# BenLangmead/bowtie2

Hardware: NVIDIA H100
Metric: Mreads/s (higher is better)
Workload: dtype u64 popcount (FM rank) + s16x2 DPX (DP)

## Files before the change

### bowtie2_b200/csrc/fm_device.cuh

```cuda
#pragma once
#include "bt2g_internal.h"

#define BT2G_OFFMASK (~(uint64_t)0)

template <typename OFF> struct SideGeom;
template <> struct SideGeom<uint32_t> {
	static constexpr uint32_t SIDE_SZ = 64, BWT_SZ = 48, BWT_LEN = 192, WORDS = 6, VECS = 4;
};
template <> struct SideGeom<uint64_t> {
	static constexpr uint32_t SIDE_SZ = 128, BWT_SZ = 96, BWT_LEN = 384, WORDS = 12, VECS = 8;
};

template <typename OFF>
struct SideRegs {
	uint64_t w[SideGeom<OFF>::WORDS];
	uint64_t occ[4];
};

__device__ __forceinline__ void ldg_sector(const uint8_t *p, uint64_t &a, uint64_t &b, uint64_t &c, uint64_t &d) {
	asm volatile("ld.global.nc.L1::no_allocate.L2::64B.v2.u64 {%0,%1}, [%4];\n\t"
	             "ld.global.nc.L1::no_allocate.L2::64B.v2.u64 {%2,%3}, [%4+16];"
	             : "=l"(a), "=l"(b), "=l"(c), "=l"(d) : "l"(p));
}
__device__ __forceinline__ void ldg_sector128(const uint8_t *p, uint64_t &a, uint64_t &b, uint64_t &c, uint64_t &d) {
// ... 203 lines not shown
		if((uint64_t)refl >= start && (uint64_t)(refl + ncol) <= start + (uint64_t)ix.recLen[lo]) {
			fast = true;
			b0 = ix.recCumUnamb[lo] + ((uint64_t)refl - start);
		}
	}
	if(fast) {
		for(int k = lane; k < ncol; k += 32) {
			const uint64_t b = b0 + (uint64_t)k;
			out[k] = (uint8_t)((ix.refBuf[b >> 2] >> ((b & 3) << 1)) & 3);
		}
	} else {
		for(int k = lane; k < ncol; k += 32) out[k] = (uint8_t)ref_base<OFF>(ix, tidx, refl + k);
	}
}

__device__ __forceinline__ int read_char(const uint8_t *seq, int len, int strand, int pos) {
	if(strand == 0) return seq[pos];
	int c = seq[len - 1 - pos];
	return c > 3 ? 4 : 3 - c;
}

template <typename OFF>
__device__ __forceinline__ uint32_t extend_one(const DevEbwt<OFF> &e, uint64_t top, uint64_t bot, const uint8_t *s, int len,
                                               int strand, int i0, int step, int lim) {
	uint32_t n = 0;
	for(int ii = 0; ii < lim; ii++) {
		const int rdc = read_char(s, len, strand, i0 + ii * step);
		if(bot - top > 1) {
			uint64_t t[4], b[4];
			rank4<OFF>(e, top, t);
			rank4<OFF>(e, bot, b);
			const uint64_t orig = bot - top;
			int nonz = -1; bool abort = false;
#pragma unroll
			for(int j = 0; j < 4; j++) {
				if(!abort && b[j] > t[j]) {
					if(nonz >= 0) abort = true;
					else { nonz = j; top = t[j]; bot = b[j]; }
				}
			}
			if(abort || (nonz != rdc && rdc <= 3) || bot - top < orig) break;
		} else {
			int c = -1;
			if(top != e.zOff) top = lf_step<OFF>(e, top, c);
			if(c != rdc && rdc <= 3) break;
			bot = top + 1;
		}
		if(++n == 255) break;
	}
	return n;
}

template <typename OFF>
__device__ __forceinline__ uint32_t extend_one_text(const DevIndex<OFF> &ix, int64_t b, int tstep, const uint8_t *s, int len,
                                                    int strand, int i0, int step, int lim) {
	uint32_t n = 0;
	const int64_t tlen = (int64_t)ix.fw.len;
	for(int ii = 0; ii < lim; ii++) {
		const int rdc = read_char(s, len, strand, i0 + ii * step);
		int c = -1;
		if(b >= 0 && b < tlen) { c = (int)((__ldg(ix.refBuf + (b >> 2)) >> ((b & 3) << 1)) & 3); b += tstep; }
		if(c != rdc && rdc <= 3) break;
		if(++n == 255) break;
	}
	return n;
}
__device__ __forceinline__ uint64_t swap_rev_pairs(uint64_t x) {
	const uint64_t y = __brevll(x);
	return ((y & 0x5555555555555555ull) << 1) | ((y >> 1) & 0x5555555555555555ull);
}
__device__ __forceinline__ uint64_t spread_bits(uint32_t m) {
	uint64_t x = m;
	x = (x | (x << 16)) & 0x0000ffff0000ffffull;
	x = (x | (x << 8)) & 0x00ff00ff00ff00ffull;
	x = (x | (x << 4)) & 0x0f0f0f0f0f0f0f0full;
	x = (x | (x << 2)) & 0x3333333333333333ull;
	x = (x | (x << 1)) & 0x5555555555555555ull;
	return x;
}
template <typename F>
__device__ __forceinline__ uint64_t walk_window(F word, int64_t p, bool asc, int64_t n, uint32_t &ok) {
	int64_t q = asc ? p : p - 31;
	int lshift = 0;
	if(q < 0) { lshift = (int)(-q); q = 0; }
	uint64_t a = 0;
	if(lshift < 32 && q < n) {
		const int64_t w = q >> 5; const int sh = (int)(q & 31);
		a = word(w) >> (2 * sh);
		if(sh && ((w + 1) << 5) < n) a |= word(w + 1) << (64 - 2 * sh);
		if(lshift) a <<= 2 * lshift;
	}
	const int64_t q0 = asc ? p : p - 31;
	uint32_t v = 0xffffffffu;
	if(q0 < 0) v = q0 <= -32 ? 0u : (v << (int)(-q0));
	if(q0 + 32 > n) { const int64_t keep = n - q0; v = keep <= 0 ? 0u : (keep >= 32 ? v : (v & ((1u << (int)keep) - 1u))); }
	if(asc) { ok = v; return a; }
	ok = __brev(v);
	return swap_rev_pairs(a);
}
template <typename OFF>
__device__ __forceinline__ uint32_t extend_one_text_packed(const DevIndex<OFF> &ix, int64_t b, int tstep, const uint64_t *pk, const uint32_t *nm, int len,
                                                           int strand, int i0, int step, int lim) {
	const int64_t tlen = (int64_t)ix.fw.len;
	const uint64_t *tw = reinterpret_cast<const uint64_t *>(ix.refBuf);
	auto tword = [&](int64_t k) -> uint64_t { return __ldg(tw + k); };
	auto rword = [&](int64_t k) -> uint64_t { return pk[k]; };
	int64_t rp = strand == 0 ? i0 : len - 1 - i0;
	const bool rasc = strand == 0 ? step > 0 : step < 0;
	const uint64_t comp = strand == 0 ? 0ull : ~0ull;
	int n = 0;
	if(lim > 255) lim = 255;
	while(n < lim) {
		uint32_t okR, okT, okN;
		const uint64_t R = walk_window(rword, rp, rasc, (int64_t)len, okR) ^ comp;
		const uint64_t T = walk_window(tword, b, tstep > 0, tlen, okT);
		uint32_t nmk;
		{
			int64_t q = rasc ? rp : rp - 31; int lshift = 0;
			if(q < 0) { lshift = (int)(-q); q = 0; }
			uint32_t a = 0;
			if(lshift < 32 && q < len) {
				const int64_t w = q >> 5; const int sh = (int)(q & 31);
				a = nm[w] >> sh;
				if(sh && ((w + 1) << 5) < len) a |= nm[w + 1] << (32 - sh);
				if(lshift) a <<= lshift;
			}
			nmk = rasc ? a : __brev(a);
			okN = 0;
		}
		(void)okN;
		const uint64_t X = R ^ T;
		const uint64_t neq = (X | (X >> 1)) & 0x5555555555555555ull;
		const uint64_t stop = (neq | spread_bits(~okT)) & ~spread_bits(nmk);
		const int chunk = lim - n < 32 ? lim - n : 32;
		int first = stop ? (__ffsll((long long)stop) - 1) >> 1 : 32;
		if(first < chunk) { n += first; break; }
		n += chunk;
		rp += rasc ? 32 : -32;
		b += tstep > 0 ? 32 : -32;
		(void)okR;
	}
	return (uint32_t)n;
}

template <typename OFF>
__device__ __forceinline__ void extend_hit(const DevIndex<OFF> &ix, const uint64_t rng[4], const uint8_t *s, int len, bool fw, int off, int sl,
                                           bool left, bool right, uint32_t &nlex, uint32_t &nrex, const uint64_t *pk = nullptr, const uint32_t *nm = nullptr) {
	const int strand = fw ? 0 : 1;
	const int limL = fw ? off : len - sl - off, limR = fw ? len - sl - off : off;
	const int i0L = fw ? off - 1 : len - off - sl - 1, i0R = fw ? sl + off : len - off;
	nlex = nrex = 0;
	const bool unique = ix.extText && ix.refBuf != nullptr && rng[1] - rng[0] == 1;
	int64_t p = 0;
	if(unique && ((left && limL > 0) || (right && limR > 0))) { unsigned ns = 0; p = (int64_t)get_offset<OFF>(ix, rng[0], ns); }
	if(left && limL > 0)
		nlex = !unique ? extend_one<OFF>(ix.fw, rng[0], rng[1], s, len, strand, i0L, -1, limL)
		     : (pk ? extend_one_text_packed<OFF>(ix, p - 1, -1, pk, nm, len, strand, i0L, -1, limL) : extend_one_text<OFF>(ix, p - 1, -1, s, len, strand, i0L, -1, limL));
	if(right && limR > 0 && ix.bw.ebwt != nullptr)
		nrex = !unique ? extend_one<OFF>(ix.bw, rng[2], rng[3], s, len, strand, i0R, +1, limR)
		     : (pk ? extend_one_text_packed<OFF>(ix, p + sl, +1, pk, nm, len, strand, i0R, +1, limR) : extend_one_text<OFF>(ix, p + sl, +1, s, len, strand, i0R, +1, limR));
}
```

### bowtie2_b200/csrc/fm_seed2.cu

```cuda
#include "fm_device.cuh"
#include <cstdlib>

#define REFILL_MIN 8

__global__ void k_pack_reads(const uint8_t *seq, const uint64_t *roff, uint64_t nReads, int maxWords,
                             uint64_t *packed, uint32_t *nmask) {
	uint64_t t = blockIdx.x * (uint64_t)blockDim.x + threadIdx.x;
	if(t >= nReads * (uint64_t)maxWords) return;
	const uint64_t rd = t / maxWords;
	const int w = (int)(t - rd * maxWords);
	const int len = (int)(roff[rd + 1] - roff[rd]);
	if(w * 32 >= len) return;
	const uint8_t *s = seq + roff[rd] + (uint64_t)w * 32;
	const int n = len - w * 32 < 32 ? len - w * 32 : 32;
	uint64_t p = 0; uint32_t m = 0;
	for(int i = 0; i < n; i++) {
		const uint32_t c = s[i];
		if(c > 3) m |= 1u << i; else p |= (uint64_t)c << (2 * i);
	}
	const uint64_t wb = (roff[rd] >> 5) + rd + (uint64_t)w;
	packed[wb] = p; nmask[wb] = m;
}

__device__ __forceinline__ uint64_t rev_pairs(uint64_t x, int n) {
	uint64_t r = __brevll(x);
	r = ((r >> 1) & 0x5555555555555555ull) | ((r & 0x5555555555555555ull) << 1);
	return r >> (64 - 2 * n);
}

template <typename OFF>
__device__ __forceinline__ void rank4_loaded(const DevEbwt<OFF> &e, const SideRegs<OFF> &s, uint64_t sideNum, uint32_t charOff, uint64_t out[4]) {
	uint32_t nC, nG, nT;
	count_cgt<OFF>(s, charOff, nC, nG, nT);
	uint32_t nA = charOff - nC - nG - nT;
	if(sideNum == e.zSide && charOff > e.zChar) nA--;
	out[0] = nA + s.occ[0] + e.fchr[0];
	out[1] = nC + s.occ[1] + e.fchr[1];
	out[2] = nG + s.occ[2] + e.fchr[2];
	out[3] = nT + s.occ[3] + e.fchr[3];
}

template <typename OFF>
__global__ void __launch_bounds__(256) k_seed_search2(DevIndex<OFF> ix, const uint64_t *packed, const uint32_t *nmask,
                                                      const uint64_t *roff, uint64_t nReads, int seedLen, int maxSeeds,
                                                      int nofw, int norc, const int32_t *interval, const int32_t *offset,
                                                      uint64_t *out, int32_t *nseedsOut, unsigned long long *next,
                                                      unsigned long long *cnt) {
	constexpr uint32_t BL = SideGeom<OFF>::BWT_LEN;
	const unsigned FULL = 0xffffffffu;
	const int lane = threadIdx.x & 31;
	const uint64_t perRead = 2ull * maxSeeds, total = nReads * perRead;
	const DevEbwt<OFF> &fw = ix.fw;
	const DevEbwt<OFF> &bw = ix.bw;
	const int ftabLen = fw.ftabChars;
	bool active = false, exhausted = false;
	uint64_t topf = 0, botf = 0, topb = 0, botb = 0, bits = 0;
	uint64_t *o = nullptr;
	int sl = 0, step = 0;
	unsigned nside = 0;
	for(;;) {
		const unsigned need = __ballot_sync(FULL, !active && !exhausted);
		if(need && (__popc(need) >= REFILL_MIN || __ballot_sync(FULL, active) == 0)) {
			unsigned long long base = 0;
			const int leader = __ffs(need) - 1;
			if(lane == leader) base = atomicAdd(next, (unsigned long long)__popc(need));
			base = __shfl_sync(FULL, base, leader);
			if(!active && !exhausted) {
				const uint64_t t = base + (unsigned)__popc(need & ((1u << lane) - 1u));
				if(t >= total) {
					exhausted = true;
				} else {
					const uint64_t rd = t / perRead;
					const int rem = (int)(t - rd * perRead);
					const int strand = rem / maxSeeds, k = rem - strand * maxSeeds;
					o = out + t * 4;
					reinterpret_cast<uint4 *>(o)[0] = make_uint4(0, 0, 0, 0);
					reinterpret_cast<uint4 *>(o)[1] = make_uint4(0, 0, 0, 0);
					const uint64_t r0 = roff[rd];
					const int len = (int)(roff[rd + 1] - r0);
					const int per = interval[rd], off0 = offset[rd];
					int nseeds = 1;
					if(len - off0 > seedLen) nseeds += (len - off0 - seedLen) / per;
					if(rem == 0 && nseedsOut) nseedsOut[rd] = nseeds;
					sl = seedLen < len ? seedLen : len;
					const int depth = k * per + off0;
					bool ok = k < nseeds && !((strand == 0 && nofw) || (strand == 1 && norc)) && depth + sl <= len && sl >= 1;
					if(ok) {
						const uint64_t wb = (r0 >> 5) + rd;
						const int w = depth >> 5, sh = depth & 31;
						const bool two = sh + sl > 32;
						const uint64_t p0 = packed[wb + w], p1 = two ? packed[wb + w + 1] : 0;
						const uint64_t n0 = nmask[wb + w], n1 = two ? nmask[wb + w + 1] : 0;
						const uint64_t m2 = sl == 32 ? ~0ull : ((1ull << (2 * sl)) - 1);
						bits = (sh ? ((p0 >> (2 * sh)) | (p1 << (64 - 2 * sh))) : p0) & m2;
						const uint64_t nb = ((n0 | (n1 << 32)) >> sh) & (sl == 32 ? 0xffffffffull : ((1ull << sl) - 1));
						if(nb) ok = false;
						if(strand == 1) bits = rev_pairs(bits, sl) ^ m2;
					}
					if(ok) {
						if(ix.ktab != nullptr && ix.ktabChars <= sl) {
							const OFF *e3 = ix.ktab + 3ull * (bits >> (2 * (sl - ix.ktabChars)));
							topf = e3[0]; botf = e3[1]; topb = e3[2]; botb = topb + (botf - topf);
							if(botf <= topf) ok = false;
							step = ix.ktabChars;
						} else if(ftabLen > 1 && ftabLen <= sl) {
							const uint64_t top20 = bits >> (2 * (sl - ftabLen));
							const uint64_t fwi = rev_pairs(top20, ftabLen), bwi = top20;
							topf = ftab_hi<OFF>(fw, fwi); botf = ftab_lo<OFF>(fw, fwi + 1);
							if(botf <= topf) ok = false;
							else if(bw.ebwt != nullptr) { topb = ftab_hi<OFF>(bw, bwi); botb = topb + (botf - topf); }
							else { topb = botb = 0; }
							step = ftabLen;
						} else {
							const int c = (int)((bits >> (2 * (sl - 1))) & 3);
							topf = topb = fw.fchr[c]; botf = botb = fw.fchr[c + 1];
							if(botf <= topf) ok = false;
							step = 1;
						}
					}
					if(ok) {
						if(step >= sl) { o[0] = topf; o[1] = botf; o[2] = topb; o[3] = botb; }
						else active = true;
					}
				}
			}
		}
		if(__ballot_sync(FULL, active) == 0) {
			if(__all_sync(FULL, exhausted)) break;
			continue;
		}
		if(active) {
			const int c = (int)((bits >> (2 * (sl - step - 1))) & 3);
			const uint64_t sideT = topf / BL, sideB = botf / BL;
			const uint32_t offT = (uint32_t)(topf - sideT * BL), offB = (uint32_t)(botf - sideB * BL);
			nside += (botf - topf > 1) ? 2 : 1;
			uint64_t tt[4], bb[4];
			SideRegs<OFF> s;
			load_side<OFF>(fw.ebwt, sideT, s);
			rank4_loaded<OFF>(fw, s, sideT, offT, tt);
			if(sideB != sideT) load_side<OFF>(fw.ebwt, sideB, s);
			rank4_loaded<OFF>(fw, s, sideB, offB, bb);
			const uint64_t w0 = bb[0] - tt[0], w1 = bb[1] - tt[1], w2 = bb[2] - tt[2];
			const uint64_t tp = topb + (c > 0 ? w0 : 0) + (c > 1 ? w1 : 0) + (c > 2 ? w2 : 0);
			const uint64_t nt = c == 0 ? tt[0] : (c == 1 ? tt[1] : (c == 2 ? tt[2] : tt[3]));
			const uint64_t nb = c == 0 ? bb[0] : (c == 1 ? bb[1] : (c == 2 ? bb[2] : bb[3]));
			if(nb <= nt) {
				active = false;
			} else {
				topf = nt; botf = nb; topb = tp; botb = tp + (nb - nt);
				if(++step == sl) { o[0] = topf; o[1] = botf; o[2] = topb; o[3] = botb; active = false; }
			}
		}
	}
	if(cnt && nside) atomicAdd(cnt, (unsigned long long)nside);
}

template <typename OFF>
__global__ void __launch_bounds__(256) k_seed_search3(DevIndex<OFF> ix, const uint64_t *packed, const uint32_t *nmask,
                                                      const uint64_t *roff, uint64_t nReads, int seedLen, int maxSeeds,
                                                      int nofw, int norc, const int32_t *interval, const int32_t *offset,
                                                      uint64_t *out, int32_t *nseedsOut, unsigned long long *next,
                                                      unsigned long long *cnt, const uint8_t *actv) {
	constexpr uint32_t BL = SideGeom<OFF>::BWT_LEN;
	const unsigned FULL = 0xffffffffu;
	const int lane = threadIdx.x & 31;
	const uint64_t total = nReads * 2;
	const DevEbwt<OFF> &fw = ix.fw;
	const DevEbwt<OFF> &bw = ix.bw;
	const int ftabLen = fw.ftabChars;
	bool haveTask = false, exhausted = false, active = false, skip = false;
	uint64_t topf = 0, botf = 0, topb = 0, botb = 0, bits = 0, wb = 0;
	uint64_t *o = nullptr, *obase = nullptr;
	int sl = 0, step = 0, k = 0, nseeds = 0, per = 1, off0 = 0, len = 0, strand = 0;
	unsigned nside = 0;
	for(;;) {
		const unsigned need = __ballot_sync(FULL, !haveTask && !exhausted);
		if(need && (__popc(need) >= REFILL_MIN || __ballot_sync(FULL, haveTask) == 0)) {
			unsigned long long base = 0;
			const int leader = __ffs(need) - 1;
			if(lane == leader) base = atomicAdd(next, (unsigned long long)__popc(need));
			base = __shfl_sync(FULL, base, leader);
			if(!haveTask && !exhausted) {
				const uint64_t t = base + (unsigned)__popc(need & ((1u << lane) - 1u));
				if(t >= total) exhausted = true;
				else if(actv && !actv[t >> 1]) { }
				else {
					const uint64_t rd = t >> 1;
					strand = (int)(t & 1);
					skip = (strand == 0 ? nofw : norc) || (actv && ((actv[rd] >> (1 + strand)) & 1));
					const uint64_t r0 = roff[rd];
					len = (int)(roff[rd + 1] - r0);
					per = interval[rd]; off0 = offset[rd];
					nseeds = 1;
					if(len - off0 > seedLen) nseeds += (len - off0 - seedLen) / per;
					if(strand == 0 && nseedsOut) nseedsOut[rd] = nseeds;
					sl = seedLen < len ? seedLen : len;
					wb = (r0 >> 5) + rd;
					obase = out + (rd * 2ull + strand) * (uint64_t)maxSeeds * 4;
					k = 0; haveTask = true; active = false;
				}
			}
		}
		if(__ballot_sync(FULL, haveTask) == 0) {
			if(__all_sync(FULL, exhausted)) break;
			continue;
		}
		if(haveTask && !active) {
			if(k >= maxSeeds) haveTask = false;
			else {
				o = obase + (uint64_t)k * 4;
				reinterpret_cast<uint4 *>(o)[0] = make_uint4(0, 0, 0, 0);
				reinterpret_cast<uint4 *>(o)[1] = make_uint4(0, 0, 0, 0);
				const int depth = k * per + off0;
				bool ok = k < nseeds && !skip && depth + sl <= len && sl >= 1;
				if(ok) {
					const int w = depth >> 5, sh = depth & 31;
					const bool two = sh + sl > 32;
					const uint64_t p0 = packed[wb + w], p1 = two ? packed[wb + w + 1] : 0;
					const uint64_t n0 = nmask[wb + w], n1 = two ? nmask[wb + w + 1] : 0;
					const uint64_t m2 = sl == 32 ? ~0ull : ((1ull << (2 * sl)) - 1);
					bits = (sh ? ((p0 >> (2 * sh)) | (p1 << (64 - 2 * sh))) : p0) & m2;
					const uint64_t nb = ((n0 | (n1 << 32)) >> sh) & (sl == 32 ? 0xffffffffull : ((1ull << sl) - 1));
					if(nb) ok = false;
					if(strand == 1) bits = rev_pairs(bits, sl) ^ m2;
				}
				if(ok) {
					if(ix.ktab != nullptr && ix.ktabChars <= sl) {
						const OFF *e3 = ix.ktab + 3ull * (bits >> (2 * (sl - ix.ktabChars)));
						topf = e3[0]; botf = e3[1]; topb = e3[2]; botb = topb + (botf - topf);
						if(botf <= topf) ok = false;
						step = ix.ktabChars;
					} else if(ftabLen > 1 && ftabLen <= sl) {
						const uint64_t top20 = bits >> (2 * (sl - ftabLen));
						const uint64_t fwi = rev_pairs(top20, ftabLen), bwi = top20;
						topf = ftab_hi<OFF>(fw, fwi); botf = ftab_lo<OFF>(fw, fwi + 1);
						if(botf <= topf) ok = false;
						else if(bw.ebwt != nullptr) { topb = ftab_hi<OFF>(bw, bwi); botb = topb + (botf - topf); }
						else { topb = botb = 0; }
						step = ftabLen;
					} else {
						const int c = (int)((bits >> (2 * (sl - 1))) & 3);
						topf = topb = fw.fchr[c]; botf = botb = fw.fchr[c + 1];
						if(botf <= topf) ok = false;
						step = 1;
					}
				}
				if(ok) {
					if(step >= sl) { o[0] = topf; o[1] = botf; o[2] = topb; o[3] = botb; }
					else active = true;
				}
				k++;
				if(!active && k >= nseeds) {
					for(; k < maxSeeds; k++) {
						uint64_t *z = obase + (uint64_t)k * 4;
						reinterpret_cast<uint4 *>(z)[0] = make_uint4(0, 0, 0, 0);
						reinterpret_cast<uint4 *>(z)[1] = make_uint4(0, 0, 0, 0);
					}
					haveTask = false;
				}
			}
		}
		if(active) {
			const int c = (int)((bits >> (2 * (sl - step - 1))) & 3);
			const uint64_t sideT = topf / BL, sideB = botf / BL;
			const uint32_t offT = (uint32_t)(topf - sideT * BL), offB = (uint32_t)(botf - sideB * BL);
			nside += (botf - topf > 1) ? 2 : 1;
			uint64_t tt[4], bb[4];
			SideRegs<OFF> s;
			load_side<OFF>(fw.ebwt, sideT, s);
			rank4_loaded<OFF>(fw, s, sideT, offT, tt);
			if(sideB != sideT) load_side<OFF>(fw.ebwt, sideB, s);
			rank4_loaded<OFF>(fw, s, sideB, offB, bb);
			const uint64_t w0 = bb[0] - tt[0], w1 = bb[1] - tt[1], w2 = bb[2] - tt[2];
			const uint64_t tp = topb + (c > 0 ? w0 : 0) + (c > 1 ? w1 : 0) + (c > 2 ? w2 : 0);
			const uint64_t nt = c == 0 ? tt[0] : (c == 1 ? tt[1] : (c == 2 ? tt[2] : tt[3]));
			const uint64_t nb = c == 0 ? bb[0] : (c == 1 ? bb[1] : (c == 2 ? bb[2] : bb[3]));
			if(nb <= nt) {
				active = false;
			} else {
				topf = nt; botf = nb; topb = tp; botb = tp + (nb - nt);
				if(++step == sl) { o[0] = topf; o[1] = botf; o[2] = topb; o[3] = botb; active = false; }
			}
		}
	}
	if(cnt && nside) atomicAdd(cnt, (unsigned long long)nside);
}

template <typename OFF>
void launch_seed_search2(const DevIndex<OFF> &ix, const uint8_t *seq, const uint64_t *roff, uint64_t nReads, int maxLen,
                         int seedLen, int maxSeeds, int nofw, int norc, const int32_t *interval, const int32_t *offset,
                         uint64_t *out, int32_t *nseeds, uint64_t *packed, uint32_t *nmask, unsigned long long *next,
                         int numSMs, cudaStream_t st, unsigned long long *cnt) {
	if(nReads == 0) return;
	(void)seq; (void)maxLen;
	cudaMemsetAsync(next, 0, sizeof(unsigned long long), st);
	int perSM = 4;
	const char *v2 = getenv("BT2G_SEED_V2");
	if(v2 && v2[0] == '1') {
		cudaOccupancyMaxActiveBlocksPerMultiprocessor(&perSM, k_seed_search2<OFF>, 256, 0);
		if(perSM < 1) perSM = 1;
		k_seed_search2<OFF><<<(unsigned)(numSMs * perSM), 256, 0, st>>>(ix, packed, nmask, roff, nReads, seedLen, maxSeeds, nofw, norc,
		                                                              interval, offset, out, nseeds, next, cnt);
		return;
	}
	cudaOccupancyMaxActiveBlocksPerMultiprocessor(&perSM, k_seed_search3<OFF>, 256, 0);
	if(perSM < 1) perSM = 1;
	k_seed_search3<OFF><<<(unsigned)(numSMs * perSM), 256, 0, st>>>(ix, packed, nmask, roff, nReads, seedLen, maxSeeds, nofw, norc,
	                                                              interval, offset, out, nseeds, next, cnt, nullptr);
}
template <typename OFF>
void launch_seed_search_active(const DevIndex<OFF> &ix, const uint64_t *roff, uint64_t nReads, int seedLen, int maxSeeds,
                               const int32_t *interval, const int32_t *offset, const uint8_t *actv, uint64_t *out, int32_t *nseeds,
                               const uint64_t *packed, const uint32_t *nmask, unsigned long long *next, int numSMs, cudaStream_t st) {
	if(nReads == 0) return;
	cudaMemsetAsync(next, 0, sizeof(unsigned long long), st);
	int perSM = 4;
	cudaOccupancyMaxActiveBlocksPerMultiprocessor(&perSM, k_seed_search3<OFF>, 256, 0);
	if(perSM < 1) perSM = 1;
	uint64_t blocks = (uint64_t)numSMs * perSM, want = (nReads * 2 + 255) / 256;
	if(want < blocks) blocks = want ? want : 1;
	k_seed_search3<OFF><<<(unsigned)blocks, 256, 0, st>>>(ix, packed, nmask, roff, nReads, seedLen, maxSeeds, 0, 0, interval, offset, out, nseeds, next, nullptr, actv);
}
template void launch_seed_search_active<uint32_t>(const DevIndex<uint32_t> &, const uint64_t *, uint64_t, int, int, const int32_t *, const int32_t *, const uint8_t *, uint64_t *, int32_t *, const uint64_t *, const uint32_t *, unsigned long long *, int, cudaStream_t);
template void launch_seed_search_active<uint64_t>(const DevIndex<uint64_t> &, const uint64_t *, uint64_t, int, int, const int32_t *, const int32_t *, const uint8_t *, uint64_t *, int32_t *, const uint64_t *, const uint32_t *, unsigned long long *, int, cudaStream_t);
template void launch_seed_search2<uint32_t>(const DevIndex<uint32_t> &, const uint8_t *, const uint64_t *, uint64_t, int, int, int, int, int, const int32_t *, const int32_t *, uint64_t *, int32_t *, uint64_t *, uint32_t *, unsigned long long *, int, cudaStream_t, unsigned long long *);
template void launch_seed_search2<uint64_t>(const DevIndex<uint64_t> &, const uint8_t *, const uint64_t *, uint64_t, int, int, int, int, int, const int32_t *, const int32_t *, uint64_t *, int32_t *, uint64_t *, uint32_t *, unsigned long long *, int, cudaStream_t, unsigned long long *);

template <typename OFF>
__global__ void k_build_ktab(DevIndex<OFF> ix, int K, OFF *out) {
	constexpr uint32_t BL = SideGeom<OFF>::BWT_LEN;
	const uint64_t x = blockIdx.x * (uint64_t)blockDim.x + threadIdx.x;
	if(x >> (2 * K)) return;
	const DevEbwt<OFF> &fw = ix.fw;
	const DevEbwt<OFF> &bw = ix.bw;
	const int F = fw.ftabChars;
	OFF *o = out + 3ull * x;
	o[0] = 0; o[1] = 0; o[2] = 0;
	const uint64_t top20 = x >> (2 * (K - F));
	const uint64_t fwi = rev_pairs(top20, F), bwi = top20;
	uint64_t topf = ftab_hi<OFF>(fw, fwi), botf = ftab_lo<OFF>(fw, fwi + 1);
	if(botf <= topf) return;
	uint64_t topb = ftab_hi<OFF>(bw, bwi);
	for(int step = F; step < K; step++) {
		const int c = (int)((x >> (2 * (K - step - 1))) & 3);
		const uint64_t sideT = topf / BL, sideB = botf / BL;
		const uint32_t offT = (uint32_t)(topf - sideT * BL), offB = (uint32_t)(botf - sideB * BL);
		uint64_t tt[4], bb[4];
		SideRegs<OFF> s;
		load_side<OFF>(fw.ebwt, sideT, s);
		rank4_loaded<OFF>(fw, s, sideT, offT, tt);
		if(sideB != sideT) load_side<OFF>(fw.ebwt, sideB, s);
		rank4_loaded<OFF>(fw, s, sideB, offB, bb);
		const uint64_t w0 = bb[0] - tt[0], w1 = bb[1] - tt[1], w2 = bb[2] - tt[2];
		const uint64_t tp = topb + (c > 0 ? w0 : 0) + (c > 1 ? w1 : 0) + (c > 2 ? w2 : 0);
		const uint64_t nt = c == 0 ? tt[0] : (c == 1 ? tt[1] : (c == 2 ? tt[2] : tt[3]));
		const uint64_t nb = c == 0 ? bb[0] : (c == 1 ? bb[1] : (c == 2 ? bb[2] : bb[3]));
		if(nb <= nt) return;
		topf = nt; botf = nb; topb = tp;
	}
	o[0] = (OFF)topf; o[1] = (OFF)botf; o[2] = (OFF)topb;
}

template <typename OFF>
void launch_build_ktab(const DevIndex<OFF> &ix, int K, OFF *out, cudaStream_t st) {
	const uint64_t n = 1ull << (2 * K);
	k_build_ktab<OFF><<<(unsigned)((n + 255) / 256), 256, 0, st>>>(ix, K, out);
}
template void launch_build_ktab<uint32_t>(const DevIndex<uint32_t> &, int, uint32_t *, cudaStream_t);
template void launch_build_ktab<uint64_t>(const DevIndex<uint64_t> &, int, uint64_t *, cudaStream_t);

template <typename OFF>
__global__ void k_build_dense_sa(DevIndex<OFF> ix, int rate, uint64_t entries, OFF *out) {
	const uint64_t i = blockIdx.x * (uint64_t)blockDim.x + threadIdx.x;
	if(i >= entries) return;
	DevIndex<OFF> base = ix;
	base.saOffs = ix.offs; base.saRate = ix.offRate;
	unsigned nside = 0;
	const uint64_t row = i << rate;
	out[i] = row < ix.fw.len + 1 ? (OFF)get_offset<OFF>(base, row, nside) : (OFF)0;
}

template <typename OFF>
void launch_build_dense_sa(const DevIndex<OFF> &ix, int rate, OFF *out, cudaStream_t st) {
	const uint64_t entries = ((ix.fw.len + 1) + ((1ull << rate) - 1)) >> rate;
	if(entries == 0) return;
	k_build_dense_sa<OFF><<<(unsigned)((entries + 255) / 256), 256, 0, st>>>(ix, rate, entries, out);
}
template void launch_build_dense_sa<uint32_t>(const DevIndex<uint32_t> &, int, uint32_t *, cudaStream_t);
template void launch_build_dense_sa<uint64_t>(const DevIndex<uint64_t> &, int, uint64_t *, cudaStream_t);

__device__ __forceinline__ int packed_char(const uint64_t *pk, const uint32_t *nm, uint64_t wb, int pos) {
	const int w = pos >> 5, b = pos & 31;
	if((nm[wb + w] >> b) & 1u) return 4;
	return (int)((pk[wb + w] >> (2 * b)) & 3);
}

template <typename OFF>
__device__ __forceinline__ uint32_t count_one(const SideRegs<OFF> &s, uint32_t charOff, int c) {
	const uint64_t M = 0x5555555555555555ull, pat = (uint64_t)c * M;
	const uint32_t wi = charOff >> 5, rem = charOff & 31;
	uint32_t n = 0;
#pragma unroll
	for(uint32_t i = 0; i < SideGeom<OFF>::WORDS; i++) {
		const uint64_t mask = i < wi ? M : (i == wi ? ((1ull << (2 * rem)) - 1) & M : 0);
		const uint64_t z = ~(s.w[i] ^ pat);
		n += __popcll(z & (z >> 1) & mask);
	}
	return n;
}

template <typename OFF>
__device__ __forceinline__ uint64_t rank1_loaded(const DevEbwt<OFF> &e, const SideRegs<OFF> &s, uint64_t sideNum, uint32_t charOff, int c) {
	uint32_t n = count_one<OFF>(s, charOff, c);
	if(c == 0 && sideNum == e.zSide && charOff > e.zChar) n--;
	const uint64_t oc = c == 0 ? s.occ[0] : (c == 1 ? s.occ[1] : (c == 2 ? s.occ[2] : s.occ[3]));
	return n + oc + e.fchr[c];
}

template <typename OFF>
__global__ void __launch_bounds__(256) k_exact_sweep2(DevIndex<OFF> ix, const uint64_t *packed, const uint32_t *nmask,
                                                      const uint64_t *roff, uint64_t nReads, int nofw, int norc,
                                                      uint8_t *mine, uint64_t *ee, unsigned long long *next, unsigned long long *cnt,
                                                      int flags) {
	const int eeOnly = flags & 1;
	const bool text = (flags & 2) != 0 && ix.refBuf != nullptr;
	constexpr uint32_t BL = SideGeom<OFF>::BWT_LEN;
	const unsigned FULL = 0xffffffffu;
	const int lane = threadIdx.x & 31;
	const uint64_t total = nReads * 2;
	const DevEbwt<OFF> &e = ix.fw;
	const int ftabLen = e.ftabChars;
	const int mineMax = 2;
	bool active = false, exhausted = false, doInit = true;
	uint64_t top = 0, bot = 0, wb = 0, task = 0;
	int len = 0, dep = 0, nedit = 0, strand = 0;
	int cacheW = -1; uint64_t cacheP = 0; uint32_t cacheM = 0;
	unsigned nside = 0;
	for(;;) {
		const unsigned need = __ballot_sync(FULL, !active && !exhausted);
		if(need && (__popc(need) >= REFILL_MIN || __ballot_sync(FULL, active) == 0)) {
			unsigned long long base = 0;
			const int leader = __ffs(need) - 1;
			if(lane == leader) base = atomicAdd(next, (unsigned long long)__popc(need));
			base = __shfl_sync(FULL, base, leader);
			if(!active && !exhausted) {
				cacheW = -1;
				task = base + (unsigned)__popc(need & ((1u << lane) - 1u));
				if(task >= total) exhausted = true;
				else {
					const uint64_t rd = task >> 1;
					strand = (int)(task & 1);
					if((strand == 0 && nofw) || (strand == 1 && norc)) {
						mine[task] = 0; ee[rd * 4 + strand * 2] = 0; ee[rd * 4 + strand * 2 + 1] = 0;
					} else {
						const uint64_t r0 = roff[rd];
						len = (int)(roff[rd + 1] - r0);
						wb = (r0 >> 5) + rd;
						dep = 0; nedit = 0; doInit = true; top = bot = 0;
						active = true;
						if(len <= 0) { mine[task] = 0; ee[rd * 4 + strand * 2] = 0; ee[rd * 4 + strand * 2 + 1] = 0; active = false; }
					}
				}
			}
		}
		if(__ballot_sync(FULL, active) == 0) {
			if(__all_sync(FULL, exhausted)) break;
			continue;
		}
		if(active) {
			bool done = false;
			auto rawchr = [&](int pos) -> int {
				const int w = pos >> 5, b = pos & 31;
				if(w != cacheW) { cacheW = w; cacheP = packed[wb + w]; cacheM = nmask[wb + w]; }
				if((cacheM >> b) & 1u) return 4;
// ... 190 lines not shown
```

### bowtie2_b200/csrc/xengine.cuh

```cuda
#pragma once
#include <stdint.h>
#include "../../include/bt2g.h"
#include "mapq_device.cuh"
#include "pe_device.cuh"

#ifndef XE_HD
#define XE_HD __host__ __device__
#endif
#define XE_HH __host__ __device__

namespace xe {

#define XE_MIN_I64 (-9223372036854775807LL - 1)
#define XE_BIG ((int64_t)1 << 62)
enum { EXHAUSTED = 1, FULFILLED, PERFECT, SOFT_LIMIT, HARD_LIMIT };
enum { XR_DONE = 0, XR_ONE_MM = 1, XR_SEED = 2, XR_DP = 3, XR_DP_MATE = 4, XR_FALLBACK = 5 };

#define XE_MAX_LEN    512
#define XE_ARENA      12288
#define XE_SEEN_IV    224
#define XE_EXR        8
#define XE_MM1        24
#define XE_MAX_SEEDS  64
#define XE_SATS       (2 * XE_MAX_SEEDS)
// ... 402 lines not shown
	}
	const int64_t sc = x_aln(u, a)->score;
	if(sc > u.usBest) { u.usBest2 = u.usBest; u.usBest = sc; } else if(sc > u.usBest2) u.usBest2 = sc;
	return u.usDone != 0;
}

XE_HD inline int64_t x_tightened(const XUnit &u, int64_t bestPairScore) {
	int64_t ps = u.best2Pair + ((u.bestPair - u.best2Pair) * 3) / 4;
	if(ps < bestPairScore) ps++;
	return ps;
}

template <typename Svc>
struct XEngine {
	const XParams &P; XUnit &u; Svc &svc;
	XE_HD XEngine(const XParams &p, XUnit &unit, Svc &s) : P(p), u(unit), svc(s) {}

	XE_HD int64_t mapq(int64_t best, bool hasSec, int64_t sec, int64_t scMin, int64_t perfect) const {
		if(!P.mmode && !hasSec) return 255;
		return mapq_v2(best, hasSec, sec, scMin, perfect, !P.local);
	}

	XE_HD int64_t shSize(const XMate &c, bool fw, int i) const { const uint64_t *h = svc.seedRange(c.idx, fw ? 0 : 1, i); return h[1] > h[0] ? (int64_t)(h[1] - h[0]) : 0; }
	XE_HD void fillSeedHits(XMate &c, int interval, int offset, int seedlen) {
		c.shN = svc.nSeeds(c.idx); c.shInterval = interval; c.shOffset = offset; c.shSeedlen = seedlen; c.shNonz = 0; c.shNelt = 0;
		if(c.shN > XE_MAX_SEEDS) { XE_FB(u); c.shN = XE_MAX_SEEDS; }
		for(int f = 0; f < 2; f++) for(int i = 0; i < c.shN; i++) { const int64_t sz = shSize(c, f == 0, i); if(sz > 0) { c.shNonz++; c.shNelt += sz; } }
	}
	XE_HD void rankSeedHits(XMate &c) {
		const int num = c.shN;
		c.nranks = 0;
		if(P.all) {
			for(int i = 1; i < num; i++) for(int f = 0; f < 2; f++) if(shSize(c, f == 0, i) > 0) c.ranks[c.nranks++] = (uint8_t)(i | (f == 0 ? 0x80 : 0));
			if(num && shSize(c, true, 0) > 0) c.ranks[c.nranks++] = 0x80;
			if(num && shSize(c, false, 0) > 0) c.ranks[c.nranks++] = 0;
			return;
		}
		uint64_t sfw = 0, src = 0;
		uint32_t szs[2][XE_MAX_SEEDS];
		for(int f = 0; f < 2; f++) for(int i = 0; i < num; i++) { const int64_t z = shSize(c, f == 0, i); szs[f][i] = z > 0xffffffffll ? 0xffffffffu : (uint32_t)z; }
		while((int64_t)c.nranks < c.shNonz) {
			uint32_t minsz = 0xffffffffu; int minidx = 0; bool minfw = true;
			const int rb = u.rnd.boolean();
			for(int fwi = 0; fwi < 2; fwi++) {
				const bool fw = fwi == (rb ? 1 : 0);
				const uint64_t srt = fw ? sfw : src;
				const uint32_t *sz = szs[fw ? 0 : 1];
				int i = (int)(u.rnd.u32() % (uint32_t)num);
				if(minsz == 1u) continue;
				for(int t = 0; t < num; t++) {
					if(sz[i] > 0 && !((srt >> i) & 1) && sz[i] < minsz) { minsz = sz[i]; minidx = i; minfw = fw; if(minsz == 1u) break; }
					if(++i == num) i = 0;
				}
			}
			if(minfw) sfw |= (uint64_t)1 << minidx; else src |= (uint64_t)1 << minidx;
			c.ranks[c.nranks++] = (uint8_t)(minidx | (minfw ? 0x80 : 0));
		}
	}

	XE_HD void addEnt(uint64_t topf, int64_t size, int rdoff, int seedlen, bool fw, int ee, bool needRand) {
		if(u.nents >= XE_ENTS) { XE_FB(u); return; }
		XEnt &e = u.ents[u.nents++];
		e.topf = topf; e.size = (int32_t)size; e.rdoff = (int16_t)rdoff; e.seedlen = (int16_t)seedlen; e.fw = fw; e.ee = (int8_t)ee; e.done1 = 0; e.mateStreak = 0;
		e.rix = 0xff;
		if(needRand && size > 1) { e.rix = (uint8_t)x_new_rand(u, (uint64_t)size, P.all != 0); if(XE_RANDS > 255 || e.rix == 0xff) XE_FB(u); }
	}
	XE_HD void eeAdd(int hi, int64_t &nelt, int64_t maxelt, bool &done) {
		const XEEHit &hit = u.hitl[hi];
		uint64_t tops[2] = {hit.top, 0}, bots[2] = {hit.bot, 0};
		const int64_t width = (int64_t)(hit.bot - hit.top);
		if(width <= 0) return;
		if(nelt + width > maxelt) {
			const int64_t trim = (nelt + width) - maxelt;
			const uint64_t rn = (P.offSize == 4 ? (uint64_t)u.rnd.u32() : u.rnd.u64()) % (uint64_t)width;
			const int64_t newwidth = width - trim;
			if(hit.top + rn + newwidth > hit.bot) { tops[0] = hit.top + rn; bots[0] = hit.bot; tops[1] = hit.top; bots[1] = hit.top + newwidth - (bots[0] - tops[0]); }
			else { tops[0] = hit.top + rn; bots[0] = tops[0] + newwidth; }
		}
		const XMate &c = u.m[u.cur];
		for(int i = 0; i < 2; i++) {
			if(done || bots[i] <= tops[i]) break;
			const int64_t w = (int64_t)(bots[i] - tops[i]);
			addEnt(tops[i], w, 0, c.rdlen, hit.fw != 0, hi, true);
			nelt += w;
			if(nelt >= maxelt) done = true;
		}
	}
	XE_HD void resetEnts() { u.nents = 0; u.nrands = 0; u.nseenPool = 0; u.nhitl = 0; }
	XE_HD void eeSaTups(bool useEe) {
		XMate &c = u.m[u.cur];
		resetEnts();
		int64_t nelt = 0; bool done = false;
		int64_t tot = 0, fwsz = 0;
		const int nee = useEe ? c.nee : 0;
		for(int i = 0; i < nee; i++) { const int64_t w = (int64_t)(c.ee[i].bot - c.ee[i].top); tot += w; if(c.ee[i].fw) fwsz += w; }
		if(tot > 0) {
			const uint64_t rn = (P.offSize == 4 ? (uint64_t)u.rnd.u32() : u.rnd.u64()) % (uint64_t)tot;
			const bool fwFirst = !((int64_t)rn >= fwsz);
			for(int fwi = 0; fwi < 2 && !done; fwi++) {
				const bool fw = (fwi == 0) == fwFirst;
				for(int i = 0; i < nee; i++) if((c.ee[i].fw != 0) == fw) { u.hitl[u.nhitl] = c.ee[i]; eeAdd(u.nhitl++, nelt, P.maxIters, done); break; }
			}
		}
		if(!done && c.nmm1 > 0) {
			for(int i = 1; i < c.nmm1; i++) { const XEEHit t = c.mm1[i]; int j = i - 1; while(j >= 0 && c.mm1[j].score < t.score) { c.mm1[j + 1] = c.mm1[j]; j--; } c.mm1[j + 1] = t; }
			{
				int streak = 0;
				for(int i = 1; i < c.nmm1; i++) {
					if(c.mm1[i].score == c.mm1[i - 1].score) { if(streak == 0) streak = 1; streak++; }
					else { if(streak > 1) x_shuffle_portion(c.mm1, i - streak, streak, u.rnd); streak = 0; }
				}
				if(streak > 1) x_shuffle_portion(c.mm1, c.nmm1 - streak, streak, u.rnd);
			}
			for(int i = 0; i < c.nmm1; i++) { if(done) break; u.hitl[u.nhitl] = c.mm1[i]; eeAdd(u.nhitl++, nelt, P.maxIters, done); }
		}
	}

	XE_HD int64_t prioritize() {
		XMate &c = u.m[u.cur];
		resetEnts();
		u.nsats = 0;
		int64_t nelt = 0;
		for(int ri = 0; ri < c.nranks; ri++) {
			const int offidx = c.ranks[ri] & 0x7f; const bool fw = (c.ranks[ri] & 0x80) != 0;
			const uint64_t *h = svc.seedRange(c.idx, fw ? 0 : 1, offidx);
			const int64_t sz = (int64_t)(h[1] - h[0]);
			const int rdoff = c.shOffset + offidx * c.shInterval, seedlen = c.shSeedlen;
			nelt += sz;
			const int st = fw ? 0 : 1;
			bool skip = false;
			for(int x = 0; x < c.nexr[st]; x++) { const XExr &e = c.exr[st][x]; if(e.p5 <= rdoff && e.p5 + e.len >= rdoff + seedlen && sz <= e.size) { skip = true; break; } }
			if(skip) { nelt -= sz; continue; }
			if(u.nsats >= XE_SATS) { XE_FB(u); break; }
			XSat &sp = u.sats[u.nsats++];
			sp.topf = h[0]; sp.topb = h[2]; sp.size = sz; sp.fw = fw; sp.offidx = (uint8_t)offidx; sp.rdoff = (int16_t)rdoff; sp.seedlen = (int16_t)seedlen;
			sp.rix = 0xff; sp.elim = 0; sp.mass = 0.0;
			int nlex = 0, nrex = 0;
			svc.extend(c.idx, fw, rdoff, seedlen, h, nlex, nrex);
			sp.nlex = (uint8_t)nlex; sp.nrex = (uint8_t)nrex;
			if(nlex > 0 || nrex > 0) {
				if(c.nexr[st] >= XE_EXR) { XE_FB(u); }
				else { XExr &e = c.exr[st][c.nexr[st]++]; e.p5 = rdoff - (fw ? nlex : nrex); e.len = seedlen + nlex + nrex; e.size = sz; }
			}
		}
		const int ns = u.nsats;
		int nsmall = 0;
		for(int i = 0; i < ns; i++) nsmall += u.sats[i].size <= 5;
		for(int i = 1; i < ns; i++) {
			const XSat t = u.sats[i]; int j = i - 1;
			while(j >= 0) {
				const XSat &b = u.sats[j];
				bool less;
				if(t.size != b.size) less = t.size < b.size;
				else if(t.topf != b.topf) less = t.topf < b.topf;
				else if(t.offidx != b.offidx) less = t.offidx < b.offidx;
				else if(t.rdoff != b.rdoff) less = t.rdoff < b.rdoff;
				else if(t.seedlen != b.seedlen) less = t.seedlen < b.seedlen;
				else less = t.fw && !b.fw;
				if(!less) break;
				u.sats[j + 1] = u.sats[j]; j--;
			}
			u.sats[j + 1] = t;
		}
		int64_t added = 0;
		int j = 0;
		while(j < nsmall && added < P.maxIters) {
			const XSat &s = u.sats[j];
			addEnt(s.topf, s.size, s.rdoff, s.seedlen, s.fw != 0, -1, true);
			added += s.size; j++;
		}
		if(added >= P.maxIters || nsmall == ns) return added;
		const int nl = ns - nsmall;
		double mass = 0.0;
		for(int i = 0; i < nl; i++) {
			XSat &s = u.sats[nsmall + i];
			double num = (double)(s.nlex + s.nrex + 1); num *= num;
			double den = (double)s.size; den *= den;
			s.mass = num / den; mass += s.mass; s.elim = 0;
		}
		while(added < P.maxIters && added < nelt) {
			const double rd = u.rnd.flt() * mass;
			double sofar = 0.0; int pick = 0, last = 0;
			bool got = false;
			for(int i = 0; i < nl; i++) if(!u.sats[nsmall + i].elim) { last = i; sofar += u.sats[nsmall + i].mass; if(rd < sofar) { pick = i; got = true; break; } }
			if(!got) pick = last;
			XSat &s = u.sats[nsmall + pick];
			if(s.rix == 0xff) { s.rix = (uint8_t)x_new_rand(u, (uint64_t)s.size, P.all != 0); }
			if(u.fallback) break;
			const uint32_t r = x_rand_next(u, s.rix, u.rnd);
			if(x_rand_done(u.rands[s.rix])) { s.elim = 1; mass -= s.mass; }
			addEnt(s.topf + r, 1, s.rdoff, s.seedlen, s.fw != 0, -1, false);
			added++;
			if(u.fallback) break;
		}
		return added;
	}
	XE_HD bool entDone(const XEnt &e) const { return e.rix == 0xff ? e.done1 != 0 : x_rand_done(u.rands[e.rix]); }
	XE_HD uint32_t entNext(XEnt &e) { if(e.rix == 0xff) { e.done1 = 1; return 0; } return x_rand_next(u, e.rix, u.rnd); }
	XE_HD void entSetDone(XEnt &e) { if(e.rix == 0xff) e.done1 = 1; else u.rands[e.rix].cur = u.rands[e.rix].n; }

	XE_HD bool dpU8(int64_t best, int64_t minsc, const XMate &mt) const {
		if(!P.local) return minsc >= -254;
		int bias = P.nPen;
		const uint8_t *q = svc.quals(mt.idx);
		for(int i = 0; i < mt.rdlen; i++) { const int p = P.mmPenalty((int)q[i] - 33); if(p > bias) bias = p; }
		return best + bias < 255;
	}
	XE_HD void reseed(bool u8) { const uint32_t rs = u.rnd.u32() + 1u; u.rnd.init(u8 ? rs + 1u : rs); }

	XE_HD bool loadAnchorDp(const XMate &c) {
		const bt2g_dp_summary *s = svc.dpSumm(u.dpSlot, false);
		u.natt = 0; u.attCursor = 0;
		if(s->flags) { XE_FB(u); return false; }
		if(!s->found) return false;
		const bt2g_dp_cand *cands = svc.dpCands(u.dpSlot, false);
		const bt2g_dp_aln *alns = svc.dpAlns(u.dpSlot, false);
		int k = 0;
		for(int ci = 0; ci < s->ncand; ci++) {
			const int f = cands[ci].fate;
			if(f != BT2G_CAND_SUCCEEDED && f != BT2G_CAND_FAILED) continue;
			if(u.natt >= XE_ATT) { XE_FB(u); return false; }
			u.attScore[u.natt] = (int16_t)cands[ci].score;
			uint16_t ao = 0xffff;
			if(f == BT2G_CAND_SUCCEEDED) {
				if(k >= svc.dpMaxAlns()) { XE_FB(u); return false; }
				ao = x_aln_from_dp(u, u.rqProb, alns[k], svc.dpOps(u.dpSlot, false, k), svc.codes(c.idx), c.rdlen);
				if(ao == 0xffff) return false;
				k++;
			}
			u.attAln[u.natt++] = ao;
		}
		u.dpU8 = dpU8(s->best, c.minsc, c);
		return true;
	}
	XE_HD bool nextAnchorAln(int64_t minsc, uint16_t &out) {
		while(u.attCursor < u.natt) {
			const int i = u.attCursor++;
			if(u.attScore[i] < minsc) continue;
			reseed(u.dpU8 != 0);
			if(u.attAln[i] != 0xffff) { out = u.attAln[i]; return true; }
		}
		return false;
	}
	XE_HD bool nextMateAln(const XMate &o, int64_t minsc, uint16_t &out) {
		const bt2g_dp_summary *s = svc.dpSumm(u.dpSlot, true);
		const bt2g_dp_cand *cands = svc.dpCands(u.dpSlot, true);
		const bt2g_dp_aln *alns = svc.dpAlns(u.dpSlot, true);
		while(u.mateCursor < s->ncand) {
			const int ci = u.mateCursor++;
			const int f = cands[ci].fate;
			if(f != BT2G_CAND_SUCCEEDED && f != BT2G_CAND_FAILED) continue;
			const bool ok = f == BT2G_CAND_SUCCEEDED;
			const int k = u.mateAlnK;
			if(ok) u.mateAlnK++;
			if(cands[ci].score < minsc) continue;
			reseed(u.odpU8 != 0);
			if(ok) {
				if(k >= svc.dpMaxAlns()) { XE_FB(u); return false; }
				out = x_aln_from_dp(u, u.rqProb, alns[k], svc.dpOps(u.dpSlot, true, k), svc.codes(o.idx), o.rdlen);
				return out != 0xffff;
			}
		}
		return false;
	}

	XE_HD void setDpReq(const XMate &c, bool fw, int64_t tidx, const XRect &rect, int64_t minsc, int rdlen) {
		bt2g_dp_problem &p = u.rqProb;
		p.read_idx = (uint32_t)c.idx; p.fw = fw ? 1u : 0u; p.tidx = (uint64_t)tidx; p.refl = rect.refl; p.refr = rect.refr;
		p.triml = (int32_t)rect.triml; p.corel = (int32_t)rect.corel; p.corer = (int32_t)rect.corer;
		p.minsc = (int32_t)minsc; p.nceil = P.nCeilRaw(rdlen); p.reserved = 0;
	}

	XE_HD int ungapped(const XMate &c, bool fw, int64_t tidx, int64_t refoff, int64_t tlen, uint16_t &out) {
		bt2g_ungapped_result r;
		const int st = svc.ungapped(c.idx, fw, tidx, refoff, tlen, c.minsc, r);
		if(st != 1) return st;
		const uint8_t *cd = svc.codes(c.idx);
		const int len = c.rdlen, rowi = r.rowi, rowf = r.rowf;
		int ned = 0;
		for(int i = rowi; i <= rowf; i++) { const int f = svc.refChar(tidx, refoff + i); if(f > 3 || x_rdchar(cd, len, fw, i) != f) ned++; }
		out = x_new_aln(u, ned);
		if(out == 0xffff) return st;
		XAln *a = x_aln(u, out);
		XEdit *ed = a->edits();
		int n = 0;
		for(int i = rowi; i <= rowf; i++) {
			const int f = svc.refChar(tidx, refoff + i), rc = x_rdchar(cd, len, fw, i);
			if(f > 3 || rc != f) { XEdit &e = ed[n++]; e.pos = (int16_t)(i - rowi); e.chr = (uint8_t)x_dna(f); e.qchr = (uint8_t)x_dna(rc); e.type = 3; e.pad = 0; }
		}
		const int tl = rowi, tr = len - 1 - rowf;
		a->tidx = (int32_t)tidx; a->refoff = refoff + rowi; a->fw = fw; a->score = r.score; a->rdlen = (int16_t)len; a->ns = (uint8_t)r.ns; a->refns = (uint8_t)r.refns;
		a->trim5 = (int16_t)(fw ? tl : tr); a->trim3 = (int16_t)(fw ? tr : tl);
		return st;
	}

	XE_HD void tightenUnpaired(XMate &c) {
		if(!(P.mmode && u.usBest2 != XE_MIN_I64)) return;
		const int64_t bot = u.usBest2 + ((u.usBest - u.usBest2) * 3) / 4;
		if(bot >= c.minsc) { c.minsc = bot; if(c.minsc < c.perfect) c.minsc++; }
	}

	XE_HD int stepExtPaired();
	XE_HD int stepExtUnpaired();
	XE_HD int stepPair();
	XE_HD int stepRead();
	XE_HD void finishPair();
	XE_HD void finishRead();
// ... 727 lines not shown
```

Before: 2.791.

## Finish unique seed matches by direct reference-text comparison instead of FM steps

When a seed's BWT range narrows to a single row during backward search, the active-seed kernel resolves that row to a text offset and checks the remaining seed characters against the packed reference. This replaces the rest of the rank steps. The offset is stored with a flag bit so downstream extension skips its own get_offset call. The satellite sort gets a tie-break for flagged rows so ordering stays deterministic. The trade-off is an extra offset lookup (an SA walk) early in the search and a change to the encoding of the seed output that downstream code must handle.

```diff
diff --git a/bowtie2_b200/csrc/fm_device.cuh b/bowtie2_b200/csrc/fm_device.cuh
--- a/bowtie2_b200/csrc/fm_device.cuh
+++ b/bowtie2_b200/csrc/fm_device.cuh
@@ -379,7 +379,10 @@
 	nlex = nrex = 0;
 	const bool unique = ix.extText && ix.refBuf != nullptr && rng[1] - rng[0] == 1;
 	int64_t p = 0;
-	if(unique && ((left && limL > 0) || (right && limR > 0))) { unsigned ns = 0; p = (int64_t)get_offset<OFF>(ix, rng[0], ns); }
+	if(unique && ((left && limL > 0) || (right && limR > 0))) {
+		unsigned ns = 0;
+		p = (rng[0] & BT2G_ROW_IS_OFFSET) ? (int64_t)(rng[0] & ~BT2G_ROW_IS_OFFSET) : (int64_t)get_offset<OFF>(ix, rng[0], ns);
+	}
 	if(left && limL > 0)
 		nlex = !unique ? extend_one<OFF>(ix.fw, rng[0], rng[1], s, len, strand, i0L, -1, limL)
 		     : (pk ? extend_one_text_packed<OFF>(ix, p - 1, -1, pk, nm, len, strand, i0L, -1, limL) : extend_one_text<OFF>(ix, p - 1, -1, s, len, strand, i0L, -1, limL));
diff --git a/bowtie2_b200/csrc/fm_seed2.cu b/bowtie2_b200/csrc/fm_seed2.cu
--- a/bowtie2_b200/csrc/fm_seed2.cu
+++ b/bowtie2_b200/csrc/fm_seed2.cu
@@ -156,11 +156,26 @@
 }
 
 template <typename OFF>
+__device__ __forceinline__ int64_t seed_text_finish(const DevIndex<OFF> &ix, uint64_t row, uint64_t bits, int r) {
+	unsigned ns = 0;
+	const int64_t q = (int64_t)get_offset<OFF>(ix, row, ns) - r;
+	if(q < 0) return -1;
+	if(r == 0) return q;
+	const uint64_t *tw = reinterpret_cast<const uint64_t *>(ix.refBuf);
+	const int64_t w = q >> 5;
+	const int sh = (int)(q & 31);
+	uint64_t a = __ldg(tw + w) >> (2 * sh);
+	if(sh + r > 32) a |= __ldg(tw + w + 1) << (64 - 2 * sh);
+	return ((a ^ bits) & ((1ull << (2 * r)) - 1)) ? -1 : q;
+}
+
+template <typename OFF>
 __global__ void __launch_bounds__(256) k_seed_search3(DevIndex<OFF> ix, const uint64_t *packed, const uint32_t *nmask,
                                                       const uint64_t *roff, uint64_t nReads, int seedLen, int maxSeeds,
                                                       int nofw, int norc, const int32_t *interval, const int32_t *offset,
                                                       uint64_t *out, int32_t *nseedsOut, unsigned long long *next,
-                                                      unsigned long long *cnt, const uint8_t *actv) {
+                                                      unsigned long long *cnt, const uint8_t *actv, int flags) {
+	const bool text = (flags & 1) != 0 && ix.refBuf != nullptr;
 	constexpr uint32_t BL = SideGeom<OFF>::BWT_LEN;
 	const unsigned FULL = 0xffffffffu;
 	const int lane = threadIdx.x & 31;
@@ -246,7 +261,10 @@
 					}
 				}
 				if(ok) {
-					if(step >= sl) { o[0] = topf; o[1] = botf; o[2] = topb; o[3] = botb; }
+					if(text && botf - topf == 1) {
+						const int64_t q = seed_text_finish<OFF>(ix, topf, bits, sl - step);
+						if(q >= 0) { o[0] = BT2G_ROW_IS_OFFSET | (uint64_t)q; o[1] = o[0] + 1; o[2] = rev_pairs(bits, sl); }
+					} else if(step >= sl) { o[0] = topf; o[1] = botf; o[2] = topb; o[3] = botb; }
 					else active = true;
 				}
 				k++;
@@ -277,6 +295,10 @@
 			const uint64_t nb = c == 0 ? bb[0] : (c == 1 ? bb[1] : (c == 2 ? bb[2] : bb[3]));
 			if(nb <= nt) {
 				active = false;
+			} else if(text && nb - nt == 1) {
+				const int64_t q = seed_text_finish<OFF>(ix, nt, bits, sl - step - 1);
+				if(q >= 0) { o[0] = BT2G_ROW_IS_OFFSET | (uint64_t)q; o[1] = o[0] + 1; o[2] = rev_pairs(bits, sl); }
+				active = false;
 			} else {
 				topf = nt; botf = nb; topb = tp; botb = tp + (nb - nt);
 				if(++step == sl) { o[0] = topf; o[1] = botf; o[2] = topb; o[3] = botb; active = false; }
@@ -306,7 +328,7 @@
 	cudaOccupancyMaxActiveBlocksPerMultiprocessor(&perSM, k_seed_search3<OFF>, 256, 0);
 	if(perSM < 1) perSM = 1;
 	k_seed_search3<OFF><<<(unsigned)(numSMs * perSM), 256, 0, st>>>(ix, packed, nmask, roff, nReads, seedLen, maxSeeds, nofw, norc,
-	                                                              interval, offset, out, nseeds, next, cnt, nullptr);
+	                                                              interval, offset, out, nseeds, next, cnt, nullptr, 0);
 }
 template <typename OFF>
 void launch_seed_search_active(const DevIndex<OFF> &ix, const uint64_t *roff, uint64_t nReads, int seedLen, int maxSeeds,
@@ -319,7 +341,8 @@
 	if(perSM < 1) perSM = 1;
 	uint64_t blocks = (uint64_t)numSMs * perSM, want = (nReads * 2 + 255) / 256;
 	if(want < blocks) blocks = want ? want : 1;
-	k_seed_search3<OFF><<<(unsigned)blocks, 256, 0, st>>>(ix, packed, nmask, roff, nReads, seedLen, maxSeeds, 0, 0, interval, offset, out, nseeds, next, nullptr, actv);
+	k_seed_search3<OFF><<<(unsigned)blocks, 256, 0, st>>>(ix, packed, nmask, roff, nReads, seedLen, maxSeeds, 0, 0, interval, offset, out, nseeds, next, nullptr, actv,
+	                                                      ix.extText ? 1 : 0 );
 }
 template void launch_seed_search_active<uint32_t>(const DevIndex<uint32_t> &, const uint64_t *, uint64_t, int, int, const int32_t *, const int32_t *, const uint8_t *, uint64_t *, int32_t *, const uint64_t *, const uint32_t *, unsigned long long *, int, cudaStream_t);
 template void launch_seed_search_active<uint64_t>(const DevIndex<uint64_t> &, const uint64_t *, uint64_t, int, int, const int32_t *, const int32_t *, const uint8_t *, uint64_t *, int32_t *, const uint64_t *, const uint32_t *, unsigned long long *, int, cudaStream_t);
diff --git a/bowtie2_b200/csrc/xengine.cuh b/bowtie2_b200/csrc/xengine.cuh
--- a/bowtie2_b200/csrc/xengine.cuh
+++ b/bowtie2_b200/csrc/xengine.cuh
@@ -578,7 +578,7 @@
 				const XSat &b = u.sats[j];
 				bool less;
 				if(t.size != b.size) less = t.size < b.size;
-				else if(t.topf != b.topf) less = t.topf < b.topf;
+				else if(t.topf != b.topf) less = ((t.topf & b.topf) >> 63) ? t.topb < b.topb : t.topf < b.topf;
 				else if(t.offidx != b.offidx) less = t.offidx < b.offidx;
 				else if(t.rdoff != b.rdoff) less = t.rdoff < b.rdoff;
 				else if(t.seedlen != b.seedlen) less = t.seedlen < b.seedlen;
```

New measurement: 2.925 (median of 6 runs). 4.8% higher.
